# pfnet/pfrl

Hardware: AMD Instinct MI355X
Metric: env-steps/sec whole node (DQN 256 envs sharded over the GPUs) (higher is better)
Workload: dtype f32

## Files before the change

include/pfrl_amd.h:

```cpp
#ifndef PFRL_AMD_H
#define PFRL_AMD_H

#include <stdint.h>

#ifdef __cplusplus
extern "C" {
#endif

#define PFRL_TAG_ABSENT 0
#define PFRL_TAG_PY 1
#define PFRL_TAG_F32 2
#define PFRL_TAG_F64 3

#define PFRL_MAX_LEVELS 40
#define PFRL_MAX_NSTEP 16
#define PFRL_MAX_STACK 8

#define PFRL_OPT_MAX_TENSORS 24

#define PFRL_POW_CORRECTLY_ROUNDED 0
#define PFRL_POW_GLIBC 1
#define PFRL_POW_GLIBC_FMA 2
#define PFRL_ERR_ARG (-2)

// ... 46 lines not shown

int pfrl_entries_append(const pfrl_table_t *tab, int64_t n_rows, const int32_t *e_slots,
                        const int32_t *tids, const int32_t *lens, void *stream);

int pfrl_batch_experiences(const pfrl_table_t *tab, const void *frames, int64_t frame_bytes,
                           int frame_is_f32, float divisor, const int32_t *entry_slots, int64_t B,
                           const double *host_gamma_pow, float *out_state, float *out_next_state,
                           void *out_action, float *out_reward, float *out_terminal,
                           float *out_discount, void *stream);

int pfrl_batch_experiences_nhwc4(const pfrl_table_t *tab, const void *frames, int64_t frame_bytes,
                                 float divisor, const int32_t *entry_slots, int64_t B,
                                 const double *host_gamma_pow, float *out_state,
                                 float *out_next_state, void *out_action, float *out_reward,
                                 float *out_terminal, float *out_discount, void *stream);

typedef struct {
    double *sum_val;
    uint8_t *sum_tag;
    double *min_val;
    uint8_t *min_tag;
    double *maxp_val;
    uint8_t *maxp_tag;
    int64_t level_off[PFRL_MAX_LEVELS];
    int64_t origin[PFRL_MAX_LEVELS];
    int64_t base;
    int64_t head;
    int64_t length;
    int32_t log2_size;
    int32_t log2_smax;
// ... 411 lines not shown
```

pfrl_amd/_native.py:

```python
import ctypes
import os
import shutil
import subprocess

_HERE = os.path.dirname(os.path.abspath(__file__))
CSRC = os.path.join(_HERE, "csrc")
LIB_DIR = os.path.join(_HERE, "lib")
LIB_PATH = os.path.join(LIB_DIR, "libpfrl_amd.so")
_LIB_OVERRIDE = os.environ.get("PFRL_AMD_LIB")
SOURCES = ["frames.hip", "replay.hip", "sumtree.hip", "rollout.hip", "optim.hip", "tdloss.hip", "operator_td.hip", "bias_act.hip", "noisy.hip", "c51.hip", "iqn.hip", "dueling.hip", "qnet.hip", "actor.hip", "actor_act.hip", "hostplan.hip", "philox.hip", "ppo_gaussian.hip", "trpo.hip", "reinforce.hip", "a2c.hip", "td3.hip"]
HIPCC_FLAGS = [
    "--offload-arch=gfx950", "-O3", "-std=c++17", "-fPIC",
    "-ffp-contract=off", "-fno-fast-math",
    "-mllvm", "-amdgpu-kernarg-preload-count=16",
    "-mllvm", "-amdgpu-mfma-vgpr-form",
]

MAX_LEVELS = 40
MAX_NSTEP = 16
MAX_STACK = 8


def _hipcc():
    for cand in (shutil.which("hipcc"), "/opt/rocm/bin/hipcc"):
# ... 103 lines not shown
    "pfrl_select_actions": (ctypes.c_int, "pippqp"),
    "pfrl_plan_sample_n_k": (ctypes.c_int, "pqip"),
    "pfrl_pyrandom_permutation": (ctypes.c_int, "pqp"),
    "pfrl_plan_eps_greedy": (ctypes.c_int, "pqdqp"),
    "pfrl_plan_dqn_range": (ctypes.c_int64, "HpqpppppPqqqiiqppqp"),
    "pfrl_batch_states_u8": (ctypes.c_int, "pqpqfpp"),
    "pfrl_batch_states_u8_nhwc4": (ctypes.c_int, "pqpqfpp"),
    "pfrl_batch_states_u8_raw_nhwc4": (ctypes.c_int, "pqpqpp"),
    "pfrl_conv2d_u8nhwc4_fwd": (ctypes.c_int, "pfpppiiiiiiiiip"),
    "pfrl_conv2d_u8nhwc4_bwd_weight": (ctypes.c_int, "pppfppqqiiiiiiiip"),
    "pfrl_batch_states_f32": (ctypes.c_int, "pqpqpp"),
    "pfrl_table_append": (ctypes.c_int, "Tqppppppp"),
    "pfrl_entries_append": (ctypes.c_int, "Tqpppp"),
    "pfrl_batch_experiences": (ctypes.c_int, "Tpqifpqpppppppp"),
    "pfrl_batch_experiences_nhwc4": (ctypes.c_int, "Tpqfpqpppppppp"),
    "pfrl_batch_episodes": (ctypes.c_int, "Tpqifpppiiqqfppppppp"),
    "pfrl_tree_write": (ctypes.c_int, "Rqppppp"),
    "pfrl_tree_write_sum": (ctypes.c_int, "Rqpppppp"),
    "pfrl_tree_update_errors_write_sample": (ctypes.c_int, "Rqppifdifdddiiqppppqpppppppppidqpp"),
    "pfrl_tree_sample": (ctypes.c_int, "Rqpppppppppidqpp"),
    "pfrl_tree_update_errors_f32": (ctypes.c_int, "Rqppifdifdddiip"),
    "pfrl_tree_update_errors_write_f32": (ctypes.c_int, "Rqppifdifdddiiqppppp"),
    "pfrl_h2d_async": (ctypes.c_int, "ppqp"),
    "pfrl_powf_host": (ctypes.c_int, "ipfpq"),
    "pfrl_powf_host_variant": (ctypes.c_int, "fq"),
    "pfrl_powf_device": (ctypes.c_int, "ipfpqp"),
    "pfrl_tree_set_priorities": (ctypes.c_int, "Rqpppip"),
    "pfrl_gae_scan": (ctypes.c_int, "qqpppppddippp"),
    "pfrl_a2c_returns": (ctypes.c_int, "qqppppddip"),
    "pfrl_adv_stats": (ctypes.c_int, "pqppp"),
# ... 160 lines not shown
```

pfrl_amd/agents/dqn.py:

```python
import collections
import copy
import os
from logging import getLogger

import numpy as np
import torch
import torch.nn.functional as F

from pfrl_amd import agent
from pfrl_amd.replay_buffer import (AbstractEpisodicReplayBuffer, DeviceExperienceBatch,
                                    ReplayUpdater, batch_experiences,
                                    batch_recurrent_experiences)
from pfrl_amd.utils.batch_states import batch_states
from pfrl_amd.utils.clip_l2_grad_norm import clip_l2_grad_norm_
from pfrl_amd.utils.contexts import evaluating
from pfrl_amd.utils.copy_param import synchronize_parameters
from pfrl_amd.utils.recurrent import (get_recurrent_state_at, mask_recurrent_state_at,
                                      one_step_forward, pack_and_forward,
                                      recurrent_state_as_numpy)


class _Pending:
    def __repr__(self):
        return "greedy(pending)"
# ... 52 lines not shown
        self._chunks.append(t)
        self._count += t.numel()
        while self._count - self._chunks[0].numel() >= self.maxlen:
            self._count -= self._chunks.popleft().numel()

    def values(self):
        if not self._chunks:
            return np.zeros(0, dtype=np.float32)
        allv = torch.cat([c.float() for c in self._chunks]).cpu().numpy()
        return allv[-self.maxlen:]

    def __len__(self):
        return min(self._count, self.maxlen)


class DQN(agent.AttributeSavingMixin, agent.BatchAgent):

    saved_attributes = ("model", "target_model", "optimizer")
    _fused_td_double = False

    def __init__(self, q_function, optimizer, replay_buffer, gamma, explorer, gpu=None,
                 replay_start_size=50000, minibatch_size=32, update_interval=1,
                 target_update_interval=10000, clip_delta=True, phi=lambda x: x,
                 target_update_method="hard", soft_update_tau=1e-2, n_times_update=1,
                 batch_accumulator="mean", episodic_update_len=None, logger=getLogger(__name__),
                 batch_states=batch_states, recurrent=False, max_grad_norm=None,
                 use_graphs=None, step_fused_gather=None, batch_target_pass=None,
                 fused_td_loss=True, replay_overlap=None, step_fused_chunks=(0.1, 0.4)):
        self.model = q_function
        if gpu is not None and gpu >= 0:
            assert torch.cuda.is_available()
            self.device = torch.device("cuda:{}".format(gpu))
            self.model.to(self.device)
            from pfrl_amd.nn.mfma_trunk import accelerate_heads

            accelerate_heads(self.model)
        else:
            self.device = torch.device("cpu")
        self.recurrent = bool(recurrent)
        if self.recurrent:
            assert isinstance(replay_buffer, AbstractEpisodicReplayBuffer)
            use_graphs = step_fused_gather = fused_td_loss = False
        self.replay_buffer = replay_buffer
# ... 37 lines not shown
        self.train_recurrent_states = None
        self.train_prev_recurrent_states = None
        self.test_recurrent_states = None
        if (self.replay_buffer.capacity is not None
                and self.replay_buffer.capacity < self.replay_updater.replay_start_size):
            raise ValueError("Replay start size cannot exceed replay buffer capacity.")
        from pfrl_amd.distributed import GradientAllReducer

        self.grad_reducer = GradientAllReducer(self.model)
        on_gpu = self.device.type == "cuda"
        self.use_graphs = on_gpu if use_graphs is None else bool(use_graphs and on_gpu)
        self.step_fused_gather = on_gpu if step_fused_gather is None else \
            bool(step_fused_gather and on_gpu)
        self.batch_target_pass = self.step_fused_gather if batch_target_pass is None else \
            bool(batch_target_pass and self.step_fused_gather)
        self.fused_td_loss = bool(fused_td_loss)
        self.step_fused_chunks = tuple(step_fused_chunks)
        self._chunks_set_by_caller = tuple(step_fused_chunks) != (0.1, 0.4)
        self._target_raw_bufs = {}
        self._single_bufs = {}
        self.range_graphs = os.environ.get("PFRL_RANGE_GRAPHS", "1") != "0"
        self.device_step = (on_gpu and self.step_fused_gather
                            and os.environ.get("PFRL_DEVICE_STEP", "1") != "0")
        self._last_actions_dev = None
        self._analytic_backward = None
        self._graphed = None
        self._last_y = None
        self._replay_stream = None
        self._fwd_event = None
        from pfrl_amd.replay_buffers.prioritized import PrioritizedReplayBuffer
# ... 115 lines not shown
                clip_l2_grad_norm_(self.model.parameters(), self.max_grad_norm)
            self.optimizer.step()
            return loss, delta
        if deferred is not None:
            deferred.append((loss, y))
        else:
            self.loss_record.extend(loss.clone())
            self.q_record.extend(y.clone())
        return loss, delta

    def _target_is_deterministic(self):
        from pfrl_amd.nn.noisy_linear import FactorizedNoisyLinear

        return not any(isinstance(m, (FactorizedNoisyLinear, torch.nn.Dropout))
                       for m in self.target_model.modules())

    def _precompute_target_raw(self, next_states):
        with torch.no_grad():
            av = self.target_model(next_states)
        if hasattr(av, "q_dist"):
            self._target_z_values = av.z_values
            return av.q_dist
        return av.q_values

    def _action_value(self, model, states, recurrent_state):
        if self.recurrent:
            return pack_and_forward(model, states, recurrent_state)[0]
        return model(states)

    def _target_next_action_value(self, exp_batch):
# ... 454 lines not shown
                j = i - lo
                if (lens[j] >= up.replay_start_size
                        and (t0 + j + 1) % up.update_interval == 0):
                    for _ in range(up.n_times_update):
                        plan_env.append(i)
                        plan_seqs.append(rbuf.lookahead_sample_at(lens[j], heads[j], up.batchsize))
        else:
            for i in range(lo, hi):
                self._append_transition(i, batch_obs, batch_reward, batch_done, batch_reset)
                if (len(rbuf) >= up.replay_start_size
                        and (t0 + (i - lo) + 1) % up.update_interval == 0):
                    for _ in range(up.n_times_update):
                        plan_env.append(i)
                        plan_seqs.append(rbuf.lookahead_sample(up.batchsize))
        if native is not None:
            big = rbuf.store.fetch_many_slots(slots_dev, U, up.batchsize, self.phi,
                                              self.gamma) if U else None
        else:
            big = rbuf.fetch_many(plan_seqs, self.phi, self.gamma) if plan_seqs else None
        if big is not None and self.batch_target_pass and self._target_is_deterministic():
            tui = self.target_update_interval
            if (t0 + (hi - lo)) // tui == t0 // tui:
                ns = big["next_state"]
                U, B = ns.shape[0], ns.shape[1]
                raw = self._precompute_target_raw(ns.view((U * B,) + tuple(ns.shape[2:])))
                key = (U, B, getattr(rbuf.store, "many_parity", 0)) + tuple(raw.shape[1:])
                buf = self._target_raw_bufs.get(key)
                if buf is None:
                    buf = self._target_raw_bufs[key] = torch.empty(
                        (U, B) + tuple(raw.shape[1:]), dtype=raw.dtype, device=raw.device)
                buf.view(raw.shape).copy_(raw)
                big["target_next_raw"] = buf
        return plan_env, big, t0

    def _run_range_updates(self, lo, hi, plan):
        plan_env, big, t0 = plan
        if big is not None and self._range_as_one_graph(t0, hi - lo):
            try:
                losses, ys = self._graphed.run_range(big)
            except Exception as e:
# ... 24 lines not shown
                mb = {k: v[p] for k, v in big.items()}
                if staged:
                    mb = self._stage_minibatch(mb)
                self._update_from_batch(mb, deferred=deferred)
                p += 1
        if deferred and self.use_graphs:
            if len({id(l) for l, _ in deferred}) == len(deferred):
                self.loss_record.extend(torch.stack([l.reshape(()) for l, _ in deferred]))
                self.q_record.extend(torch.cat([y.reshape(-1) for _, y in deferred]))
            else:
                for l, y in deferred:
                    self.loss_record.extend(l.clone())
                    self.q_record.extend(y.clone())

    def _stage_minibatch(self, mb):
        key = tuple(sorted((k, tuple(v.shape), v.dtype, v.stride()) for k, v in mb.items()))
        bufs = self._single_bufs.get(key)
        if bufs is None:
            bufs = self._single_bufs[key] = {k: torch.empty_strided(v.shape, v.stride(), dtype=v.dtype,
                                                                    device=v.device)
                                             for k, v in mb.items()}
        for k, v in mb.items():
            bufs[k].copy_(v)
        return bufs

    def _batched_append_ok(self, lo, hi, batch_obs):
        from pfrl_amd.device_store import DeviceObsBatch

        prev = getattr(self, "_last_obs_batch", None)
        rbuf = self.replay_buffer
        return (not self.recurrent and isinstance(batch_obs, DeviceObsBatch)
                and isinstance(prev, DeviceObsBatch) and prev.store is batch_obs.store
                and len(prev) == len(batch_obs)
                and hasattr(rbuf, "batch_append_supported") and rbuf.batch_append_supported(batch_obs)
                and all(o is not None for o in self.batch_last_obs[lo:hi]))

    def _range_as_one_graph(self, t0, n):
        if not (self.use_graphs and self.range_graphs):
# ... 70 lines not shown
```

pfrl_amd/agents/graphed_update.py:

```python
import collections
import gc
import logging
import os

import torch

from pfrl_amd import distributed


def _capture_kwargs(pool):
    kw = {} if pool is None else {"pool": pool}
    kw["capture_error_mode"] = "thread_local"
    return kw


class _capturing:

    def __init__(self, g, pool):
        self.ctx = torch.cuda.graph(g, **_capture_kwargs(pool))

    def __enter__(self):
        self.was_enabled = gc.isenabled()
        r = self.ctx.__enter__()
        gc.disable()
# ... 100 lines not shown

    def __init__(self, agent, max_graphs=256):
        self.agent = agent
        self.graphs = _GraphCache(max_graphs)
        self.pool = None
        self.enabled = True
        self.max_graphs = max_graphs
        self.logger = logging.getLogger(__name__)
        self._capturable_done = False
        self.split_for_allreduce = (distributed.world_size() > 1
                                    or os.environ.get("PFRL_FORCE_SPLIT_GRAPH") == "1")
        self.pipeline = False
        self.graph_collective = os.environ.get("PFRL_GRAPH_COLLECTIVE", "auto")

    def _key(self, exp_batch):
        return (tuple(sorted((k, v.data_ptr(), tuple(v.shape)) for k, v in exp_batch.items()
                             if isinstance(v, torch.Tensor))),
                _hyper_signature([self.agent.optimizer]))

    def _forward(self, exp_batch, want_errors):
        ag = self.agent
        ag._analytic_backward = None
        ag._defer_head_fold = not self.pipeline
        from pfrl_amd.nn import mfma_trunk

        del mfma_trunk._DEFERRED_FOLDS[:]
        try:
            return ag._compute_loss(exp_batch, want_errors=want_errors, record=False)
        finally:
            ag._defer_head_fold = False

# ... 623 lines not shown
```

pfrl_amd/csrc/nhwc.h:

```cpp
#pragma once
#include <hip/hip_runtime.h>
#include <stdint.h>

namespace pfrl_nhwc {

constexpr int kTilePixels = 1024;

__device__ __forceinline__ int tiles_per_obs(int64_t npix) {
    return (int)((npix + kTilePixels - 1) / kTilePixels);
}

template <bool DIV, bool NT>
__device__ __forceinline__ void convert_tile(const uint8_t *__restrict__ f0,
                                             const uint8_t *__restrict__ f1,
                                             const uint8_t *__restrict__ f2,
                                             const uint8_t *__restrict__ f3,
                                             float4 *__restrict__ dst_obs, int tile, int npix,
                                             float d) {
    __shared__ uint32_t s_raw[4][256];
    const int tid = threadIdx.x;
    const int px0 = tile * kTilePixels;
    const int ndw = min(256, (npix - px0) >> 2);
    const int i = (px0 >> 2) + min(tid, ndw - 1);
    const uint32_t w0 = reinterpret_cast<const uint32_t *>(f0)[i];
// ... 22 lines not shown
                o.w = __fdiv_rn(o.w, d);
            }
            float4 *dst = dst_obs + px0 + p;
            if (NT) {
                __builtin_nontemporal_store(o.x, &dst->x);
                __builtin_nontemporal_store(o.y, &dst->y);
                __builtin_nontemporal_store(o.z, &dst->z);
                __builtin_nontemporal_store(o.w, &dst->w);
            } else {
                *dst = o;
            }
        }
    }
}

}
```

pfrl_amd/csrc/replay.hip:

```cpp
#include <hip/hip_ext.h>

#include <stdlib.h>

#include <vector>

#include "common.h"
#include "nhwc.h"

namespace {

constexpr int kThreads = 256;
constexpr int kUnroll = 8;

struct TimedLaunch {
    hipEvent_t start, stop;
    int64_t units;
    int32_t kind;
};
bool g_profile = false;
std::vector<TimedLaunch> g_timed;

struct GammaPow {
    double g[PFRL_MAX_NSTEP + 1];
};
// ... 185 lines not shown
    }
    const int64_t r = (f - 2 * nf) * kThreads + threadIdx.x;
    if (r >= ea.rows) return;
    const int step = upper_index(ea.row_start, ea.T, r);
    const int b = (int)(r - ea.row_start[step]);
    const int64_t es = ((int64_t)ea.ep_first[b] + step) % ea.E;
    const int64_t t = tab.e_tids[es * tab.n];
    out_reward[r] = (float)tab.t_reward[t];
    out_terminal[r] = tab.t_terminal[t] != 0 ? 1.0f : 0.0f;
    out_discount[r] = gamma;
    const int ad = tab.act_dim > 0 ? tab.act_dim : 1;
    const ActT *src = reinterpret_cast<const ActT *>(tab.t_action);
    for (int i = 0; i < ad; ++i) out_action[r * ad + i] = src[t * ad + i];
}

template <int MODE, typename ActT, bool NT>
__global__ __launch_bounds__(kThreads) void k_batch_experiences_nhwc4(
    pfrl_table_t tab, const uint8_t *__restrict__ frames, int64_t frame_bytes, float divisor,
    const int32_t *__restrict__ entry_slots, int64_t B, GammaPow gp, uint8_t *__restrict__ out_state,
    uint8_t *__restrict__ out_next, ActT *__restrict__ out_action, float *__restrict__ out_reward,
    float *__restrict__ out_terminal, float *__restrict__ out_discount, int tiles) {
    const int64_t nt_blocks = 2 * B * tiles;
    const int64_t scalar_blocks = (int64_t)gridDim.x - nt_blocks;
    if ((int64_t)blockIdx.x >= scalar_blocks) {
        const int64_t tb = (int64_t)blockIdx.x - scalar_blocks;
        const int64_t ot = tb / tiles;
        const int tile = (int)(tb - ot * tiles);
        const bool is_next = ot >= B;
        const int64_t b = is_next ? ot - B : ot;
        const int64_t e = entry_slots[b];
        const int32_t *r;
        if (!is_next) {
            r = tab.t_state_ref + (int64_t)tab.e_tids[e * tab.n] * 4;
        } else {
            const int len = tab.e_len[e];
            r = tab.t_next_ref + (int64_t)tab.e_tids[e * tab.n + len - 1] * 4;
        }
        const uint8_t *f0 = frames + (int64_t)r[0] * frame_bytes;
        const uint8_t *f1 = frames + (int64_t)r[1] * frame_bytes;
        const uint8_t *f2 = frames + (int64_t)r[2] * frame_bytes;
        const uint8_t *f3 = frames + (int64_t)r[3] * frame_bytes;
        float4 *dst = reinterpret_cast<float4 *>((is_next ? out_next : out_state) +
                                                 b * 16 * frame_bytes);
        pfrl_nhwc::convert_tile<MODE == 0, NT>(f0, f1, f2, f3, dst, tile, (int)frame_bytes,
                                               divisor);
        return;
    }
    const int64_t b = (int64_t)blockIdx.x * kThreads + threadIdx.x;
    if (b >= B) return;
    const int64_t e = entry_slots[b];
    const int len = tab.e_len[e];
    double acc = 0.0;
    bool any = false;
    for (int i = 0; i < len; ++i) {
        const int64_t t = tab.e_tids[e * tab.n + i];
        acc = __dadd_rn(acc, __dmul_rn(gp.g[i], tab.t_reward[t]));
// ... 214 lines not shown
        (void)hipEventSynchronize(t.stop);
        float ms = 0.0f;
        if (hipEventElapsedTime(&ms, t.start, t.stop) == hipSuccess && n < cap) {
            out_us[n] = (double)ms * 1e3;
            out_units[n] = t.units;
            out_kind[n] = t.kind;
            ++n;
        }
        (void)hipEventDestroy(t.start);
        (void)hipEventDestroy(t.stop);
    }
    g_timed.clear();
    return n;
}

template <int MODE, bool NT>
static void launch_be_nhwc4(const pfrl_table_t *tab, const void *frames, int64_t frame_bytes,
                            float divisor, const int32_t *entry_slots, int64_t B,
                            const GammaPow &gp, float *out_state, float *out_next_state,
                            void *out_action, float *out_reward, float *out_terminal,
                            float *out_discount, hipStream_t stream) {
    const int tiles = (int)((frame_bytes + pfrl_nhwc::kTilePixels - 1) / pfrl_nhwc::kTilePixels);
    const unsigned blocks = (unsigned)(2 * B * tiles + (B + kThreads - 1) / kThreads);
    hipEvent_t e0 = nullptr, e1 = nullptr;
    pfrl_profile_events(PFRL_PROFILE_BATCH_EXPERIENCES, B, &e0, &e1);
    if (tab->act_dim > 0)
        hipExtLaunchKernelGGL((k_batch_experiences_nhwc4<MODE, float, NT>), dim3(blocks),
                              dim3(kThreads), 0, stream, e0, e1, 0, *tab, (const uint8_t *)frames,
                              frame_bytes, divisor, entry_slots, B, gp, (uint8_t *)out_state,
                              (uint8_t *)out_next_state, (float *)out_action, out_reward,
                              out_terminal, out_discount, tiles);
    else
        hipExtLaunchKernelGGL((k_batch_experiences_nhwc4<MODE, int64_t, NT>), dim3(blocks),
                              dim3(kThreads), 0, stream, e0, e1, 0, *tab, (const uint8_t *)frames,
                              frame_bytes, divisor, entry_slots, B, gp, (uint8_t *)out_state,
                              (uint8_t *)out_next_state, (int64_t *)out_action, out_reward,
                              out_terminal, out_discount, tiles);
}

extern "C" int pfrl_batch_experiences_nhwc4(const pfrl_table_t *tab, const void *frames,
                                            int64_t frame_bytes, float divisor,
                                            const int32_t *entry_slots, int64_t B,
                                            const double *host_gamma_pow, float *out_state,
                                            float *out_next_state, void *out_action,
                                            float *out_reward, float *out_terminal,
                                            float *out_discount, void *stream) {
    PFRL_CHECK_ARG(tab && tab->k == 4, "pfrl_batch_experiences_nhwc4: stacks of 4 frames only");
    PFRL_CHECK_ARG(tab->n >= 1 && tab->n <= PFRL_MAX_NSTEP, "bad table.n");
// ... 13 lines not shown
                                      out_state, out_next_state, out_action, out_reward,
                                      out_terminal, out_discount, s);
    } else {
        if (nt)
            launch_be_nhwc4<0, true>(tab, frames, frame_bytes, divisor, entry_slots, B, gp,
                                     out_state, out_next_state, out_action, out_reward,
                                     out_terminal, out_discount, s);
        else
            launch_be_nhwc4<0, false>(tab, frames, frame_bytes, divisor, entry_slots, B, gp,
                                      out_state, out_next_state, out_action, out_reward,
                                      out_terminal, out_discount, s);
    }
    PFRL_LAUNCH_CHECK();
}

extern "C" int pfrl_batch_episodes(const pfrl_table_t *tab, const void *frames, int64_t frame_bytes,
                                   int frames_are_f32, float divisor, const int32_t *ep_first,
                                   const int32_t *ep_row0, const int32_t *row_start, int32_t n_eps,
                                   int32_t T, int64_t rows, int64_t entry_ring, float gamma,
                                   void *out_state, void *out_next_state, void *out_action,
                                   float *out_reward, float *out_terminal, float *out_discount,
                                   void *stream) {
    PFRL_CHECK_ARG(tab && tab->n >= 1 && tab->k >= 1 && tab->k <= PFRL_MAX_STACK, "bad table");
    PFRL_CHECK_ARG(frame_bytes > 0 && (frame_bytes & 3) == 0, "frame_bytes must be a multiple of 4");
    PFRL_CHECK_ARG(n_eps >= 1 && T >= 1 && rows >= 1 && entry_ring >= 1 && ep_first && ep_row0 &&
                       row_start, "pfrl_batch_episodes: bad episode table");
    EpisodeArgs ea{ep_first, ep_row0, row_start, n_eps, T, rows, entry_ring};
    const int64_t frame_blocks = 2 * rows * tab->k;
    const dim3 grid((unsigned)(frame_blocks + (rows + kThreads - 1) / kThreads)), block(kThreads);
    hipStream_t st = (hipStream_t)stream;
// ... 16 lines not shown
```

pfrl_amd/nn/atari_cnn.py:

```python
import torch
import torch.nn as nn
import torch.nn.functional as F

from pfrl_amd.initializers import init_chainer_default


def constant_bias_initializer(bias=0.0):
    @torch.no_grad()
    def init_bias(m):
        if isinstance(m, (nn.Linear, nn.Conv2d)):
            m.bias.fill_(bias)

    return init_bias


def wants_channels_last(model):
    for m in model.modules():
        if isinstance(m, nn.Conv2d):
            w = m.weight
            return (w.dim() == 4 and w.is_contiguous(memory_format=torch.channels_last)
                    and not w.is_contiguous())
    return False


# ... 54 lines not shown
    def forward(self, x):
        return conv_activation(self, x, F.relu)


class _AtariCNN(nn.Module):
    def __init__(self, convs, flat, n_output_channels, activation, bias):
        super().__init__()
        self.activation = activation
        self.n_output_channels = n_output_channels
        self.layers = nn.ModuleList(convs)
        self.output = nn.Linear(flat, n_output_channels)
        self.apply(init_chainer_default)
        self.apply(constant_bias_initializer(bias=bias))

    def forward(self, state):
        if _is_relu(self.activation) and state.is_cuda:
            from pfrl_amd.nn import mfma_trunk

            specs = mfma_trunk.plan_for(self.layers, self.output, state)
            if specs is not None:
                return mfma_trunk.trunk_forward(state, specs, list(self.layers), self.output)
        h = state
        last = len(self.layers) - 1
        for i, layer in enumerate(self.layers):
            h = conv_activation(layer, h, self.activation, planar_out=(i == last))
        return linear_activation(self.output, h.reshape(h.size(0), -1), self.activation)


class LargeAtariCNN(_AtariCNN):

# ... 16 lines not shown
```

pfrl_amd/nn/mfma_trunk.py:

```python
import contextlib
import ctypes
import os

import torch
import torch.nn as nn

from pfrl_amd import _native
from pfrl_amd._native import check

_ENABLED = os.environ.get("PFRL_MFMA_TRUNK", "1") != "0"
_MAX_BATCH = int(os.environ.get("PFRL_MFMA_TRUNK_MAX_BATCH", "0"))
SMALL_LINEAR_MAX_OUT = 16


_raw_stream = getattr(torch._C, "_cuda_getCurrentRawStream", None)


def _stream():
    if _raw_stream is not None:
        return ctypes.c_void_p(_raw_stream(torch.cuda.current_device()))
    return ctypes.c_void_p(torch.cuda.current_stream().cuda_stream)


def _p(t):
# ... 40 lines not shown
            and conv.out_channels % 32 == 0 and conv.out_channels % 64 != 0
            and H >= conv.kernel_size[0] and W >= conv.kernel_size[1]):
        return False
    st = conv.stride[0]
    M = max(M, _PLAN_BATCH)
    rows = M * ((H - conv.kernel_size[0]) // st + 1) * ((W - conv.kernel_size[1]) // st + 1)
    return (_ceil_div(rows, 32) * (conv.out_channels // 32) >= 384
            and ops.u8_division_exact(divisor))


def u8_first_layer_ok(conv, px):
    d = px.data
    return (d.is_cuda and d.dtype == torch.uint8 and d.dim() == 4 and d.shape[3] == 4
            and d.is_contiguous() and d.data_ptr() % 16 == 0
            and u8_first_layer_shape_ok(conv, d.shape[0], d.shape[1], d.shape[2], px.divisor))


_U8_FIRST = os.environ.get("PFRL_U8_CONV1", "1") != "0"


def plan_for(convs, linear, x):
    from pfrl_amd.ops import U8Pixels

    if isinstance(x, U8Pixels):
        if not (_ENABLED and _native.available() and convs and u8_first_layer_ok(convs[0], x)):
            return None
    elif not (_ENABLED and x.is_cuda and x.dtype == torch.float32 and x.dim() == 4
              and not x.requires_grad and _native.available()):
        return None
    if _MAX_BATCH and x.shape[0] > _MAX_BATCH:
# ... 567 lines not shown
```

pfrl_amd/ops.py:

```python
import ctypes
import os

import numpy as np
import torch

from pfrl_amd import _native
from pfrl_amd._native import TableDesc, check


_raw_stream = getattr(torch._C, "_cuda_getCurrentRawStream", None)


def _stream():
    if _raw_stream is not None:
        return ctypes.c_void_p(_raw_stream(torch.cuda.current_device()))
    return ctypes.c_void_p(torch.cuda.current_stream().cuda_stream)


def _ptr(t):
    if t is None:
        return None
    assert t.is_cuda and t.is_contiguous(), "device-contiguous tensor required"
    return ctypes.c_void_p(t.data_ptr())

# ... 145 lines not shown
    check(_native.lib().pfrl_batch_states_u8_nhwc4(
        _ptr(frames), frame_bytes_of(frames), _ptr(refs), M, float(divisor),
        ctypes.c_void_p(out.data_ptr()), _stream()), "batch_states_u8_nhwc4")
    return out


class U8Pixels:

    __slots__ = ("data", "divisor")

    def __init__(self, data, divisor):
        self.data, self.divisor = data, float(divisor)

    @property
    def shape(self):
        M, H, W, C = self.data.shape
        return torch.Size((M, C, H, W))

    @property
    def device(self):
        return self.data.device

    def float(self):
        lut = torch.from_numpy(np.arange(256, dtype=np.float32) / np.float32(self.divisor))
        return lut.to(self.data.device)[self.data.long()].permute(0, 3, 1, 2)


_U8_DIV_OK = {}


def u8_division_exact(divisor):
    d32 = np.float32(divisor)
    key = float(d32)
    hit = _U8_DIV_OK.get(key)
    if hit is not None:
        return hit
    from fractions import Fraction as Fr

    def rn(fr):
        f = np.float32(float(fr))
# ... 107 lines not shown
    kinds = (ctypes.c_int32 * cap)()
    n = _native.lib().pfrl_profile_collect(us, ent, kinds, cap)
    if kind is None:
        return list(us[:n]), list(ent[:n]), list(kinds[:n])
    sel = [i for i in range(n) if kinds[i] == kind]
    return [us[i] for i in sel], [ent[i] for i in sel]


def batch_experiences(desc, frames, divisor, entry_slots, gamma_pow, out):
    B = entry_slots.numel()
    gp = (ctypes.c_double * len(gamma_pow))(*gamma_pow)
    st = out["state"]
    if st.dim() == 4 and not st.is_contiguous() and \
            st.is_contiguous(memory_format=torch.channels_last):
        assert channels_last_supported(frames, desc.k)
        assert out["next_state"].is_contiguous(memory_format=torch.channels_last)
        check(_native.lib().pfrl_batch_experiences_nhwc4(
            ctypes.byref(desc), _ptr(frames), frame_bytes_of(frames), float(divisor),
            _ptr(entry_slots), B, ctypes.cast(gp, ctypes.c_void_p),
            ctypes.c_void_p(st.data_ptr()), ctypes.c_void_p(out["next_state"].data_ptr()),
            _ptr(out["action"]), _ptr(out["reward"]), _ptr(out["is_state_terminal"]),
            _ptr(out["discount"]), _stream()), "batch_experiences_nhwc4")
        return out
    check(_native.lib().pfrl_batch_experiences(
        ctypes.byref(desc), _ptr(frames), frame_bytes_of(frames),
        int(frames.dtype == torch.float32), float(divisor), _ptr(entry_slots), B,
        ctypes.cast(gp, ctypes.c_void_p), _ptr(out["state"]), _ptr(out["next_state"]),
        _ptr(out["action"]), _ptr(out["reward"]), _ptr(out["is_state_terminal"]),
        _ptr(out["discount"]), _stream()), "batch_experiences")
    return out
# ... 1133 lines not shown
```

pfrl_amd/replay_buffers/device_replay.py:

```python
import collections

import numpy as np
import torch

from pfrl_amd import ops
from pfrl_amd.device_store import DeviceFrameStore, DeviceObs, recognise_phi
from pfrl_amd.staging import StagingRing, on_stream

_STAGE_ROWS = 4096


class _LazyFramesLike:
    """Duck type of pfrl.wrappers.atari_wrappers.LazyFrames: ``_frames`` list."""


def _frames_of(obs):
    fr = getattr(obs, "_frames", None)
    if isinstance(fr, (list, tuple)) and len(fr) > 0:
        return fr
    return None


class DeviceReplayStore:
    MANY_SETS = int(__import__("os").environ.get("PFRL_MANY_SETS", "2"))
# ... 514 lines not shown
                if sample.shape[0] == 1:
                    sample = sample[0]
                elif sample.ndim >= 3 and sample.shape[1] == 1:
                    sample = np.concatenate(list(sample), axis=0)
                if not np.any(sample):
                    sample = sample.copy()
                    sample.reshape(-1)[: 256] = np.arange(min(256, sample.size), dtype=np.uint8)
            d = recognise_phi(phi, sample)
            if d is None:
                raise TypeError(
                    "pfrl_amd: phi is not a cast/scale feature extractor and the observations "
                    "are already device-resident; use phi(x) = float32(x) / c")
            self._divisor = d
        return self._divisor

    def _out_buffers(self, B, tag):
        nhwc = bool(self.frames.emit_channels_last
                    and ops.channels_last_supported(self.frames.frames, self.k))
        key = (tag, B, nhwc)
        out = self._out_cache.get(key)
        if out is not None:
            return out
        dev = self.device
        fshape = self.frames.frame_shape
        k = self.k
        if k == 1:
            oshape = (B,) + fshape
        elif len(fshape) >= 2 and fshape[0] == 1:
            oshape = (B, k) + fshape[1:]
        else:
            oshape = (B, k) + fshape
        if nhwc:
            hw = oshape[-2:]
            new_obs = lambda: ops.empty_channels_last(B, hw, dev)
        else:
            new_obs = lambda: torch.empty(oshape, dtype=torch.float32, device=dev)
        out = dict(
            state=new_obs(),
            next_state=new_obs(),
            action=(torch.empty(B, dtype=torch.int64, device=dev) if self.act_dim == 0 else
                    torch.empty((B, self.act_dim), dtype=torch.float32, device=dev)),
            reward=torch.empty(B, dtype=torch.float32, device=dev),
            is_state_terminal=torch.empty(B, dtype=torch.float32, device=dev),
            discount=torch.empty(B, dtype=torch.float32, device=dev),
        )
        self._out_cache[key] = out
        return out

    def fetch(self, batch, phi, gamma):
        self.flush()
        B = len(batch)
        tag = "single"
        if self.double_buffer:
            self._out_parity ^= 1
# ... 13 lines not shown
        return out

    def fetch_many(self, seq_sets, phi, gamma):
        self.flush()
        U = len(seq_sets)
        B = len(seq_sets[0])
        seqs = np.concatenate(seq_sets)
        slots_dev = self.slots_for(seqs)
        flat = self._out_buffers(U * B, "many")
        gp = [gamma ** i for i in range(self.n + 1)]
        with on_stream(self.side_stream):
            ops.batch_experiences(self.desc, self.frames.frames, self.divisor_for(phi), slots_dev,
                                  gp, flat)
        return {k: v.view((U, B) + tuple(v.shape[1:])) for k, v in flat.items()}

    def fetch_many_slots(self, slots_dev, U, B, phi, gamma, alternate=True):
        self.flush()
        if not alternate:
            flat = self._out_buffers(U * B, "many")
            gp = [gamma ** i for i in range(self.n + 1)]
            with on_stream(self.side_stream):
                ops.batch_experiences(self.desc, self.frames.frames, self.divisor_for(phi),
                                      slots_dev, gp, flat)
            return {k: v.view((U, B) + tuple(v.shape[1:])) for k, v in flat.items()}
        self.many_parity = (self.many_parity + 1) % self.MANY_SETS
        flat = self._out_buffers(U * B, "many%d" % self.many_parity)
        gp = [gamma ** i for i in range(self.n + 1)]
        with on_stream(self.side_stream):
            ops.batch_experiences(self.desc, self.frames.frames, self.divisor_for(phi), slots_dev,
                                  gp, flat)
        key = (U, B, id(flat))
        views = self._many_views.get(key)
        if views is None or views[0] is not flat:
            if len(self._many_views) > 16:
                self._many_views.clear()
            views = self._many_views[key] = (
                flat, {k: v.view((U, B) + tuple(v.shape[1:])) for k, v in flat.items()})
        return dict(views[1])

    def fetch_episodes(self, windows, phi, gamma):
        self.flush()
        n = len(windows)
        lens = np.array([w[1] for w in windows], dtype=np.int64)
        assert n > 0 and lens.min() >= 1 and (lens[:-1] >= lens[1:]).all()
        rows, T = int(lens.sum()), int(lens[0])
        ep_first = np.array([w[0] % self.E for w in windows], dtype=np.int32)
        ep_row0 = np.zeros(n + 1, dtype=np.int32)
        ep_row0[1:] = np.cumsum(lens)
        row_start = np.minimum(lens[None, :], np.arange(T + 1)[:, None]).sum(axis=1).astype(np.int32)
        if self.frames is not None:
            oldest = min(int(self.h_e_min_fseq[(w[0] + np.arange(w[1])) % self.E].min())
                         for w in windows)
# ... 125 lines not shown
```

Before: 42240.

## Emit next-state observations as packed uint8 NHWC4 for the target pass

When the target network's first layer can consume uint8 pixels, the replay gather kernel packs next-state frame stacks into uint8 NHWC4 instead of expanding them to f32. The target pass then feeds these into the u8-entry conv trunk through a U8Pixels wrapper, which cuts the bytes written and read for next states by four. Supporting plumbing covers U8Pixels indexing and reshaping, graph keying, minibatch staging and a cached LUT. The route is guarded by many eligibility checks, and the path is complex enough that a fallback mismatch or a subclass reading next_state could hit the slow float() conversion.

```diff
diff --git a/include/pfrl_amd.h b/include/pfrl_amd.h
--- a/include/pfrl_amd.h
+++ b/include/pfrl_amd.h
@@ -84,6 +84,13 @@
                                  const double *host_gamma_pow, float *out_state,
                                  float *out_next_state, void *out_action, float *out_reward,
                                  float *out_terminal, float *out_discount, void *stream);
+
+int pfrl_batch_experiences_nhwc4_next_u8(const pfrl_table_t *tab, const void *frames,
+                                         int64_t frame_bytes, float divisor,
+                                         const int32_t *entry_slots, int64_t B,
+                                         const double *host_gamma_pow, float *out_state,
+                                         void *out_next_u8, void *out_action, float *out_reward,
+                                         float *out_terminal, float *out_discount, void *stream);
 
 typedef struct {
     double *sum_val;
diff --git a/pfrl_amd/_native.py b/pfrl_amd/_native.py
--- a/pfrl_amd/_native.py
+++ b/pfrl_amd/_native.py
@@ -141,6 +141,7 @@
     "pfrl_entries_append": (ctypes.c_int, "Tqpppp"),
     "pfrl_batch_experiences": (ctypes.c_int, "Tpqifpqpppppppp"),
     "pfrl_batch_experiences_nhwc4": (ctypes.c_int, "Tpqfpqpppppppp"),
+    "pfrl_batch_experiences_nhwc4_next_u8": (ctypes.c_int, "Tpqfpqpppppppp"),
     "pfrl_batch_episodes": (ctypes.c_int, "Tpqifpppiiqqfppppppp"),
     "pfrl_tree_write": (ctypes.c_int, "Rqppppp"),
     "pfrl_tree_write_sum": (ctypes.c_int, "Rqpppppp"),
diff --git a/pfrl_amd/agents/dqn.py b/pfrl_amd/agents/dqn.py
--- a/pfrl_amd/agents/dqn.py
+++ b/pfrl_amd/agents/dqn.py
@@ -90,6 +90,12 @@
         return min(self._count, self.maxlen)
 
 
+def next_states_as_u8(*, allowed, batch_target_pass, target_deterministic, first_layer_ok,
+                      frames_u8_k4, next_state_read_elsewhere):
+    return bool(allowed and batch_target_pass and target_deterministic and first_layer_ok
+                and frames_u8_k4 and not next_state_read_elsewhere)
+
+
 class DQN(agent.AttributeSavingMixin, agent.BatchAgent):
 
     saved_attributes = ("model", "target_model", "optimizer")
@@ -102,7 +108,8 @@
                  batch_accumulator="mean", episodic_update_len=None, logger=getLogger(__name__),
                  batch_states=batch_states, recurrent=False, max_grad_norm=None,
                  use_graphs=None, step_fused_gather=None, batch_target_pass=None,
-                 fused_td_loss=True, replay_overlap=None, step_fused_chunks=(0.1, 0.4)):
+                 fused_td_loss=True, replay_overlap=None, step_fused_chunks=(0.1, 0.4),
+                 u8_next_states=True):
         self.model = q_function
         if gpu is not None and gpu >= 0:
             assert torch.cuda.is_available()
@@ -170,6 +177,7 @@
             bool(step_fused_gather and on_gpu)
         self.batch_target_pass = self.step_fused_gather if batch_target_pass is None else \
             bool(batch_target_pass and self.step_fused_gather)
+        self.u8_next_states = bool(u8_next_states)
         self.fused_td_loss = bool(fused_td_loss)
         self.step_fused_chunks = tuple(step_fused_chunks)
         self._chunks_set_by_caller = tuple(step_fused_chunks) != (0.1, 0.4)
@@ -315,6 +323,36 @@
 
         return not any(isinstance(m, (FactorizedNoisyLinear, torch.nn.Dropout))
                        for m in self.target_model.modules())
+
+    _next_state_readers = ("_compute_target_values", "_target_next_action_value",
+                           "_compute_y_and_t", "_compute_loss", "_compute_loss_fused",
+                           "_precompute_target_raw", "_action_value", "_graphed_step",
+                           "_update_from_batch", "update")
+
+    def _reads_next_state_elsewhere(self):
+        cls = type(self)
+        return not (cls._fused_td_double is False and not cls._operator_td_stock
+                    and not self.recurrent
+                    and all(getattr(cls, n) is getattr(DQN, n) for n in self._next_state_readers))
+
+    def _next_u8_route(self, store, rows):
+        from pfrl_amd import ops
+        from pfrl_amd.nn import mfma_trunk
+
+        fr = getattr(store, "frames", None)
+        frames_ok = bool(
+            fr is not None and fr.frames.dtype == torch.uint8 and store.k == 4
+            and fr.emit_channels_last and ops.channels_last_supported(fr.frames, 4))
+        first_ok = False
+        if frames_ok and self.u8_next_states:
+            conv = mfma_trunk.u8_entry_conv(self.target_model)
+            hw = fr.frames.shape[-2:]
+            first_ok = conv is not None and mfma_trunk.u8_first_layer_shape_ok(
+                conv, rows, hw[0], hw[1], store.divisor_for(self.phi))
+        return next_states_as_u8(
+            allowed=self.u8_next_states, batch_target_pass=self.batch_target_pass,
+            target_deterministic=self._target_is_deterministic(), first_layer_ok=first_ok,
+            frames_u8_k4=frames_ok, next_state_read_elsewhere=self._reads_next_state_elsewhere())
 
     def _precompute_target_raw(self, next_states):
         with torch.no_grad():
@@ -799,6 +837,8 @@
                         plan_env.append(i)
                         plan_seqs.append(rbuf.lookahead_sample(up.batchsize))
         if native is not None:
+            if U:
+                rbuf.store.next_states_u8 = self._next_u8_route(rbuf.store, U * up.batchsize)
             big = rbuf.store.fetch_many_slots(slots_dev, U, up.batchsize, self.phi,
                                               self.gamma) if U else None
         else:
@@ -808,7 +848,11 @@
             if (t0 + (hi - lo)) // tui == t0 // tui:
                 ns = big["next_state"]
                 U, B = ns.shape[0], ns.shape[1]
-                raw = self._precompute_target_raw(ns.view((U * B,) + tuple(ns.shape[2:])))
+                if torch.is_tensor(ns):
+                    ns = ns.view((U * B,) + tuple(ns.shape[2:]))
+                else:
+                    ns = ns.rows(U * B)
+                raw = self._precompute_target_raw(ns)
                 key = (U, B, getattr(rbuf.store, "many_parity", 0)) + tuple(raw.shape[1:])
                 buf = self._target_raw_bufs.get(key)
                 if buf is None:
@@ -863,6 +907,10 @@
                     self.q_record.extend(y.clone())
 
     def _stage_minibatch(self, mb):
+        from pfrl_amd.ops import U8Pixels
+
+        px = {k: v for k, v in mb.items() if isinstance(v, U8Pixels)}
+        mb = {k: (v.data if k in px else v) for k, v in mb.items()}
         key = tuple(sorted((k, tuple(v.shape), v.dtype, v.stride()) for k, v in mb.items()))
         bufs = self._single_bufs.get(key)
         if bufs is None:
@@ -871,6 +919,8 @@
                                              for k, v in mb.items()}
         for k, v in mb.items():
             bufs[k].copy_(v)
+        if px:
+            return {k: (U8Pixels(v, px[k].divisor) if k in px else v) for k, v in bufs.items()}
         return bufs
 
     def _batched_append_ok(self, lo, hi, batch_obs):
diff --git a/pfrl_amd/agents/graphed_update.py b/pfrl_amd/agents/graphed_update.py
--- a/pfrl_amd/agents/graphed_update.py
+++ b/pfrl_amd/agents/graphed_update.py
@@ -138,7 +138,10 @@
         self.graph_collective = os.environ.get("PFRL_GRAPH_COLLECTIVE", "auto")
 
     def _key(self, exp_batch):
-        return (tuple(sorted((k, v.data_ptr(), tuple(v.shape)) for k, v in exp_batch.items()
+        from pfrl_amd.ops import U8Pixels
+
+        vals = ((k, v.data if isinstance(v, U8Pixels) else v) for k, v in exp_batch.items())
+        return (tuple(sorted((k, v.data_ptr(), tuple(v.shape)) for k, v in vals
                              if isinstance(v, torch.Tensor))),
                 _hyper_signature([self.agent.optimizer]))
 
diff --git a/pfrl_amd/csrc/nhwc.h b/pfrl_amd/csrc/nhwc.h
--- a/pfrl_amd/csrc/nhwc.h
+++ b/pfrl_amd/csrc/nhwc.h
@@ -60,4 +60,35 @@
     }
 }
 
+template <bool NT>
+__device__ __forceinline__ void pack_tile_u8(const uint8_t *__restrict__ f0,
+                                             const uint8_t *__restrict__ f1,
+                                             const uint8_t *__restrict__ f2,
+                                             const uint8_t *__restrict__ f3,
+                                             uint4 *__restrict__ dst_obs, int tile, int npix) {
+    const int tid = threadIdx.x;
+    const int px0 = tile * kTilePixels;
+    const int ndw = min(256, (npix - px0) >> 2);
+    if (tid >= ndw) return;
+    const int i = (px0 >> 2) + tid;
+    const uint32_t w0 = reinterpret_cast<const uint32_t *>(f0)[i];
+    const uint32_t w1 = reinterpret_cast<const uint32_t *>(f1)[i];
+    const uint32_t w2 = reinterpret_cast<const uint32_t *>(f2)[i];
+    const uint32_t w3 = reinterpret_cast<const uint32_t *>(f3)[i];
+    uint4 o;
+    o.x = (w0 & 0xffu) | ((w1 & 0xffu) << 8) | ((w2 & 0xffu) << 16) | (w3 << 24);
+    o.y = ((w0 >> 8) & 0xffu) | (w1 & 0xff00u) | ((w2 & 0xff00u) << 8) | ((w3 & 0xff00u) << 16);
+    o.z = ((w0 >> 16) & 0xffu) | ((w1 >> 8) & 0xff00u) | (w2 & 0xff0000u) | ((w3 & 0xff0000u) << 8);
+    o.w = (w0 >> 24) | ((w1 >> 16) & 0xff00u) | ((w2 >> 8) & 0xff0000u) | (w3 & 0xff000000u);
+    uint4 *dst = dst_obs + i;
+    if (NT) {
+        __builtin_nontemporal_store(o.x, &dst->x);
+        __builtin_nontemporal_store(o.y, &dst->y);
+        __builtin_nontemporal_store(o.z, &dst->z);
+        __builtin_nontemporal_store(o.w, &dst->w);
+    } else {
+        *dst = o;
+    }
 }
+
+}
diff --git a/pfrl_amd/csrc/replay.hip b/pfrl_amd/csrc/replay.hip
--- a/pfrl_amd/csrc/replay.hip
+++ b/pfrl_amd/csrc/replay.hip
@@ -223,7 +223,7 @@
     for (int i = 0; i < ad; ++i) out_action[r * ad + i] = src[t * ad + i];
 }
 
-template <int MODE, typename ActT, bool NT>
+template <int MODE, typename ActT, bool NT, bool NEXT_U8 = false>
 __global__ __launch_bounds__(kThreads) void k_batch_experiences_nhwc4(
     pfrl_table_t tab, const uint8_t *__restrict__ frames, int64_t frame_bytes, float divisor,
     const int32_t *__restrict__ entry_slots, int64_t B, GammaPow gp, uint8_t *__restrict__ out_state,
@@ -249,6 +249,12 @@
         const uint8_t *f1 = frames + (int64_t)r[1] * frame_bytes;
         const uint8_t *f2 = frames + (int64_t)r[2] * frame_bytes;
         const uint8_t *f3 = frames + (int64_t)r[3] * frame_bytes;
+        if (NEXT_U8 && is_next) {
+            pfrl_nhwc::pack_tile_u8<NT>(f0, f1, f2, f3,
+                                        reinterpret_cast<uint4 *>(out_next + b * 4 * frame_bytes),
+                                        tile, (int)frame_bytes);
+            return;
+        }
         float4 *dst = reinterpret_cast<float4 *>((is_next ? out_next : out_state) +
                                                  b * 16 * frame_bytes);
         pfrl_nhwc::convert_tile<MODE == 0, NT>(f0, f1, f2, f3, dst, tile, (int)frame_bytes,
@@ -493,10 +499,10 @@
     return n;
 }
 
-template <int MODE, bool NT>
+template <int MODE, bool NT, bool NEXT_U8 = false>
 static void launch_be_nhwc4(const pfrl_table_t *tab, const void *frames, int64_t frame_bytes,
                             float divisor, const int32_t *entry_slots, int64_t B,
-                            const GammaPow &gp, float *out_state, float *out_next_state,
+                            const GammaPow &gp, float *out_state, void *out_next_state,
                             void *out_action, float *out_reward, float *out_terminal,
                             float *out_discount, hipStream_t stream) {
     const int tiles = (int)((frame_bytes + pfrl_nhwc::kTilePixels - 1) / pfrl_nhwc::kTilePixels);
@@ -504,13 +510,13 @@
     hipEvent_t e0 = nullptr, e1 = nullptr;
     pfrl_profile_events(PFRL_PROFILE_BATCH_EXPERIENCES, B, &e0, &e1);
     if (tab->act_dim > 0)
-        hipExtLaunchKernelGGL((k_batch_experiences_nhwc4<MODE, float, NT>), dim3(blocks),
+        hipExtLaunchKernelGGL((k_batch_experiences_nhwc4<MODE, float, NT, NEXT_U8>), dim3(blocks),
                               dim3(kThreads), 0, stream, e0, e1, 0, *tab, (const uint8_t *)frames,
                               frame_bytes, divisor, entry_slots, B, gp, (uint8_t *)out_state,
                               (uint8_t *)out_next_state, (float *)out_action, out_reward,
                               out_terminal, out_discount, tiles);
     else
-        hipExtLaunchKernelGGL((k_batch_experiences_nhwc4<MODE, int64_t, NT>), dim3(blocks),
+        hipExtLaunchKernelGGL((k_batch_experiences_nhwc4<MODE, int64_t, NT, NEXT_U8>), dim3(blocks),
                               dim3(kThreads), 0, stream, e0, e1, 0, *tab, (const uint8_t *)frames,
                               frame_bytes, divisor, entry_slots, B, gp, (uint8_t *)out_state,
                               (uint8_t *)out_next_state, (int64_t *)out_action, out_reward,
@@ -554,6 +560,35 @@
     PFRL_LAUNCH_CHECK();
 }
 
+extern "C" int pfrl_batch_experiences_nhwc4_next_u8(
+    const pfrl_table_t *tab, const void *frames, int64_t frame_bytes, float divisor,
+    const int32_t *entry_slots, int64_t B, const double *host_gamma_pow, float *out_state,
+    void *out_next_u8, void *out_action, float *out_reward, float *out_terminal,
+    float *out_discount, void *stream) {
+    PFRL_CHECK_ARG(tab && tab->k == 4,
+                   "pfrl_batch_experiences_nhwc4_next_u8: stacks of 4 frames only");
+    PFRL_CHECK_ARG(tab->n >= 1 && tab->n <= PFRL_MAX_NSTEP, "bad table.n");
+    PFRL_CHECK_ARG(frame_bytes > 0 && (frame_bytes & 3) == 0, "frame_bytes must be a multiple of 4");
+    PFRL_CHECK_ARG(((uintptr_t)out_next_u8 & 15) == 0,
+                   "pfrl_batch_experiences_nhwc4_next_u8: out_next_u8 must be 16-byte aligned");
+    if (B <= 0) return 0;
+    GammaPow gp;
+    for (int i = 0; i <= tab->n; ++i) gp.g[i] = host_gamma_pow[i];
+    hipStream_t s = (hipStream_t)stream;
+    const bool nt = 2 * B * 16 * frame_bytes >= kNtMinBytes;
+#define BE_U8(MODE, NT)                                                                          \
+    launch_be_nhwc4<MODE, NT, true>(tab, frames, frame_bytes, divisor, entry_slots, B, gp,       \
+                                    out_state, out_next_u8, out_action, out_reward,              \
+                                    out_terminal, out_discount, s)
+    if (divisor == 1.0f) {
+        if (nt) BE_U8(1, true); else BE_U8(1, false);
+    } else {
+        if (nt) BE_U8(0, true); else BE_U8(0, false);
+    }
+#undef BE_U8
+    PFRL_LAUNCH_CHECK();
+}
+
 extern "C" int pfrl_batch_episodes(const pfrl_table_t *tab, const void *frames, int64_t frame_bytes,
                                    int frames_are_f32, float divisor, const int32_t *ep_first,
                                    const int32_t *ep_row0, const int32_t *row_start, int32_t n_eps,
diff --git a/pfrl_amd/nn/atari_cnn.py b/pfrl_amd/nn/atari_cnn.py
--- a/pfrl_amd/nn/atari_cnn.py
+++ b/pfrl_amd/nn/atari_cnn.py
@@ -92,6 +92,16 @@
         self.apply(constant_bias_initializer(bias=bias))
 
     def forward(self, state):
+        from pfrl_amd.ops import U8Pixels
+
+        if isinstance(state, U8Pixels):
+            from pfrl_amd.nn import mfma_trunk
+
+            specs = mfma_trunk.plan_for(self.layers, self.output, state) \
+                if _is_relu(self.activation) else None
+            if specs is not None:
+                return mfma_trunk.trunk_forward(state, specs, list(self.layers), self.output)
+            state = state.float()
         if _is_relu(self.activation) and state.is_cuda:
             from pfrl_amd.nn import mfma_trunk
 
diff --git a/pfrl_amd/nn/mfma_trunk.py b/pfrl_amd/nn/mfma_trunk.py
--- a/pfrl_amd/nn/mfma_trunk.py
+++ b/pfrl_amd/nn/mfma_trunk.py
@@ -78,6 +78,19 @@
     return (d.is_cuda and d.dtype == torch.uint8 and d.dim() == 4 and d.shape[3] == 4
             and d.is_contiguous() and d.data_ptr() % 16 == 0
             and u8_first_layer_shape_ok(conv, d.shape[0], d.shape[1], d.shape[2], px.divisor))
+
+
+def u8_entry_conv(model):
+    from pfrl_amd.nn.atari_cnn import _AtariCNN, _is_relu
+
+    m = model
+    while type(m) is nn.Sequential and len(m) > 0:
+        m = m[0]
+    if isinstance(m, _AtariCNN) and _is_relu(m.activation) and len(m.layers) > 0:
+        return m.layers[0]
+    if isinstance(m, _TrunkSequential) and m._trunk_run[0] == 0:
+        return list(m._modules.values())[m._trunk_run[2][0]]
+    return None
 
 
 _U8_FIRST = os.environ.get("PFRL_U8_CONV1", "1") != "0"
diff --git a/pfrl_amd/ops.py b/pfrl_amd/ops.py
--- a/pfrl_amd/ops.py
+++ b/pfrl_amd/ops.py
@@ -183,16 +183,37 @@
 
     @property
     def shape(self):
-        M, H, W, C = self.data.shape
-        return torch.Size((M, C, H, W))
+        *lead, H, W, C = self.data.shape
+        return torch.Size(tuple(lead) + (C, H, W))
 
     @property
     def device(self):
         return self.data.device
 
+    @property
+    def is_cuda(self):
+        return self.data.is_cuda
+
+    def __getitem__(self, index):
+        assert self.data.dim() > 4 or isinstance(index, slice)
+        return U8Pixels(self.data[index], self.divisor)
+
+    def rows(self, *lead):
+        return U8Pixels(self.data.view(tuple(lead) + tuple(self.data.shape[-3:])), self.divisor)
+
     def float(self):
-        lut = torch.from_numpy(np.arange(256, dtype=np.float32) / np.float32(self.divisor))
-        return lut.to(self.data.device)[self.data.long()].permute(0, 3, 1, 2)
+        key = (self.data.device, self.divisor)
+        lut = _U8_LUT.get(key)
+        if lut is None:
+            lut = torch.from_numpy(np.arange(256, dtype=np.float32) / np.float32(self.divisor))
+            lut = _U8_LUT[key] = lut.to(self.data.device)
+        return lut[self.data.long()].movedim(-1, -3)
+
+    def detach(self):
+        return self.float()
+
+
+_U8_LUT = {}
 
 
 _U8_DIV_OK = {}
@@ -330,6 +351,18 @@
     if st.dim() == 4 and not st.is_contiguous() and \
             st.is_contiguous(memory_format=torch.channels_last):
         assert channels_last_supported(frames, desc.k)
+        nxt = out["next_state"]
+        if isinstance(nxt, U8Pixels):
+            assert frames.dtype == torch.uint8 and nxt.divisor == float(divisor)
+            assert nxt.data.dtype == torch.uint8 and nxt.data.is_contiguous() and \
+                tuple(nxt.data.shape) == (B,) + tuple(st.shape[2:]) + (4,)
+            check(_native.lib().pfrl_batch_experiences_nhwc4_next_u8(
+                ctypes.byref(desc), _ptr(frames), frame_bytes_of(frames), float(divisor),
+                _ptr(entry_slots), B, ctypes.cast(gp, ctypes.c_void_p),
+                ctypes.c_void_p(st.data_ptr()), ctypes.c_void_p(nxt.data.data_ptr()),
+                _ptr(out["action"]), _ptr(out["reward"]), _ptr(out["is_state_terminal"]),
+                _ptr(out["discount"]), _stream()), "batch_experiences_nhwc4_next_u8")
+            return out
         assert out["next_state"].is_contiguous(memory_format=torch.channels_last)
         check(_native.lib().pfrl_batch_experiences_nhwc4(
             ctypes.byref(desc), _ptr(frames), frame_bytes_of(frames), float(divisor),
diff --git a/pfrl_amd/replay_buffers/device_replay.py b/pfrl_amd/replay_buffers/device_replay.py
--- a/pfrl_amd/replay_buffers/device_replay.py
+++ b/pfrl_amd/replay_buffers/device_replay.py
@@ -552,10 +552,10 @@
             self._divisor = d
         return self._divisor
 
-    def _out_buffers(self, B, tag):
+    def _out_buffers(self, B, tag, next_u8_divisor=None):
         nhwc = bool(self.frames.emit_channels_last
                     and ops.channels_last_supported(self.frames.frames, self.k))
-        key = (tag, B, nhwc)
+        key = (tag, B, nhwc) if next_u8_divisor is None else (tag, B, nhwc, float(next_u8_divisor))
         out = self._out_cache.get(key)
         if out is not None:
             return out
@@ -573,9 +573,16 @@
             new_obs = lambda: ops.empty_channels_last(B, hw, dev)
         else:
             new_obs = lambda: torch.empty(oshape, dtype=torch.float32, device=dev)
+        if next_u8_divisor is None:
+            new_next = new_obs
+        else:
+            assert nhwc and self.frames.dtype == torch.uint8 and k == 4
+            new_next = lambda: ops.U8Pixels(
+                torch.empty((B,) + tuple(oshape[-2:]) + (4,), dtype=torch.uint8, device=dev),
+                next_u8_divisor)
         out = dict(
             state=new_obs(),
-            next_state=new_obs(),
+            next_state=new_next(),
             action=(torch.empty(B, dtype=torch.int64, device=dev) if self.act_dim == 0 else
                     torch.empty((B, self.act_dim), dtype=torch.float32, device=dev)),
             reward=torch.empty(B, dtype=torch.float32, device=dev),
@@ -619,17 +626,24 @@
                                   gp, flat)
         return {k: v.view((U, B) + tuple(v.shape[1:])) for k, v in flat.items()}
 
+    next_states_u8 = False
+
     def fetch_many_slots(self, slots_dev, U, B, phi, gamma, alternate=True):
         self.flush()
+        u8_div = self.divisor_for(phi) if self.next_states_u8 else None
+
+        def split(v):
+            return v.rows(U, B) if isinstance(v, ops.U8Pixels) else v.view((U, B) + tuple(v.shape[1:]))
+
         if not alternate:
-            flat = self._out_buffers(U * B, "many")
+            flat = self._out_buffers(U * B, "many", u8_div)
             gp = [gamma ** i for i in range(self.n + 1)]
             with on_stream(self.side_stream):
                 ops.batch_experiences(self.desc, self.frames.frames, self.divisor_for(phi),
                                       slots_dev, gp, flat)
-            return {k: v.view((U, B) + tuple(v.shape[1:])) for k, v in flat.items()}
+            return {k: split(v) for k, v in flat.items()}
         self.many_parity = (self.many_parity + 1) % self.MANY_SETS
-        flat = self._out_buffers(U * B, "many%d" % self.many_parity)
+        flat = self._out_buffers(U * B, "many%d" % self.many_parity, u8_div)
         gp = [gamma ** i for i in range(self.n + 1)]
         with on_stream(self.side_stream):
             ops.batch_experiences(self.desc, self.frames.frames, self.divisor_for(phi), slots_dev,
@@ -639,8 +653,7 @@
         if views is None or views[0] is not flat:
             if len(self._many_views) > 16:
                 self._many_views.clear()
-            views = self._many_views[key] = (
-                flat, {k: v.view((U, B) + tuple(v.shape[1:])) for k, v in flat.items()})
+            views = self._many_views[key] = (flat, {k: split(v) for k, v in flat.items()})
         return dict(views[1])
 
     def fetch_episodes(self, windows, phi, gamma):
```

New measurement: 42540, median of 6. Within noise of the previous version (+0.7%).
